# wagnva/semantic-nerf-for-satellite-data

Measured on AMD Instinct MI355X. Metric: train rays/sec (4096 rays x 64 samples), higher is better.
Workload: dtype f32(f16x2)

## Files before the change

### semantic-nerf-for-satellite-data_amd/csrc/bsp.h

```cpp
#pragma once
#include "common.h"
#include "gemm.h"

namespace snerf {
namespace bsp {

constexpr int RB = 128;
constexpr int CB = 128;
constexpr int E_MAX = 100;
constexpr int E_QUIET = 60;

typedef __amdgpu_buffer_rsrc_t srd_t;
typedef unsigned int u32x4 __attribute__((ext_vector_type(4)));
typedef unsigned int u32x2 __attribute__((ext_vector_type(2)));
typedef _Float16 f16x8 __attribute__((ext_vector_type(8)));
typedef _Float16 f16x4 __attribute__((ext_vector_type(4)));
constexpr unsigned OOB = 0xFFFFFFF0u;

__host__ __device__ inline int ncb_of(int ld) { return (ld + CB - 1) / CB; }
__host__ __device__ inline size_t plane_bytes(size_t rows, int ld, int pl = 2) { return rows * (size_t)ld * 2 * pl; }
__host__ __device__ inline size_t etab_ints(size_t rows, int ld) { return ((rows + RB - 1) / RB) * (size_t)ncb_of(ld); }
__host__ __device__ inline unsigned g16_off(int k, int pl = 2) { return (unsigned)(k >> 4) * 32u * (unsigned)pl + (unsigned)(k & 15) * 2u; }

__host__ __device__ inline int exp_of_maxbits(unsigned b) {
// ... 66 lines not shown
  const char* W = nullptr;
  const int* EW = nullptr;
  int w_rb32 = 0, w_row0 = 0, w_k0 = 0; unsigned w_bytes = 0;
  int I = 0, J = 0, K = 0;
  char* C = nullptr; int* EC = nullptr; int ldc = 0; int c_col0 = 0;
  float* Cf = nullptr;
  const float* bias = nullptr;
  int act = ACT_NONE; float w0 = 1.f;
  unsigned* Csign = nullptr;
  int aux_mode = AUX_NONE;
  const char* H = nullptr; const int* EH = nullptr; int ldh = 0; int h_col0 = 0; const unsigned* Hsign = nullptr;
  float* colsum = nullptr; int ldcs = 0;
  int tiles_i = 0, tiles_j = 0;
  int tj_skip = -1;
  int tiles_jr = 0;
  int rev = 0;
  int dbg = 0;
  int* tile_ctr = nullptr;
  int pl = 2;
  const float* nd_w = nullptr; float* nd_out = nullptr; unsigned long long nd_stride = 0;
  int nd_omax = 0, nd_ldw = 0;
  int nd_rows[8] = {0, 0, 0, 0, 0, 0, 0, 0}, nd_row0[8] = {0, 0, 0, 0, 0, 0, 0, 0}, nd_woff[8] = {0, 0, 0, 0, 0, 0, 0, 0};
};
__host__ __device__ inline size_t sign_words(size_t rows, int ld) { return ((rows + 31) / 32) * (size_t)((ld + 63) / 64) * 64; }

struct DwArgs {
  const char* A = nullptr; const int* EA = nullptr; int lda = 0; int a_col0 = 0;
  const char* B = nullptr; const int* EB = nullptr; int ldb = 0; int b_col0 = 0;
  int I = 0, J = 0, P = 0;
  float* C = nullptr; int ldc = 0;
  int k_split = 0, n_split = 1; unsigned long long slab_stride = 0;
  int tiles_i = 0, tiles_j = 0;
  int pl = 2;
};

constexpr int TR_MAXL = 8;
constexpr int TR_SLOTS = TR_MAXL + 1;
struct TrunkArgs {
  const char* pe = nullptr; const int* Epe = nullptr;
  int P = 0, W = 0, L = 0; unsigned skip_mask = 0;
  int gamma_free_layer = 0;
  const char* Wp[TR_SLOTS] = {}; const int* EW[TR_SLOTS] = {}; unsigned w_bytes[TR_SLOTS] = {}; int K[TR_SLOTS] = {};
  const float* bias[TR_SLOTS] = {}; float w0[TR_SLOTS] = {};
  char* F = nullptr; int* EF = nullptr; int ldf = 0;
  char* H[TR_MAXL] = {}; int* EH[TR_MAXL] = {}; unsigned* Hsign[TR_MAXL] = {};
  const float* nd_w = nullptr; float* nd_out = nullptr; unsigned long long nd_stride = 0;
  int* tile_ctr = nullptr;
  int dbg = 0;
};
inline int trunk_gamma_free_layer(int L, unsigned skip_mask) {
  int g = 2;
  for (int l = 2; l < L; ++l)
    if ((skip_mask >> l) & 1u) g = l;
  return g < L - 1 ? g : L - 1;
}
inline bool trunk_dma_in_final_layer(int L, unsigned skip_mask, bool feats_fused) {
  return !feats_fused && trunk_gamma_free_layer(L, skip_mask) == L - 1;
}
int launch_trunk(const TrunkArgs& a, bool train, hipStream_t st);
void trunk_set_grid_override(int n);
void trunk_set_fusion(int on);
bool trunk_fusion_enabled();

int launch_kc(const KcArgs& a, hipStream_t st);
void kc_set_grid_override(int n);
int launch_kc_narrow(const KcArgs& a, hipStream_t st);
// ... 48 lines not shown
```

### semantic-nerf-for-satellite-data_amd/csrc/bsp_gemm.hip

```cpp
#include "bsp_dev.h"

#include <vector>

namespace snerf {
namespace bsp {

constexpr int KC_STRIP = 32 * 68 * 4;
constexpr int KN_A = 128 * 64, KN_RING = 4, KN_TAIL = KN_RING * KN_A, KN_LDS = KN_TAIL + 512;

template <int PL>
__global__ __launch_bounds__(256, 4) void gemm_kcn_kernel(const KcArgs p) {
  constexpr int EB = 2 * PL, KSUB = PL == 2 ? 16 : 32, KSH = PL == 2 ? 4 : 5;
  __shared__ __attribute__((aligned(16))) char lds[KN_LDS];
  int* etab = reinterpret_cast<int*>(lds + KN_TAIL);
  const int t = threadIdx.x, lane = t & 63;
  const int wave = __builtin_amdgcn_readfirstlane(t >> 6);
  const int ti = blockIdx.x, i0 = ti * 128, wi0 = wave * 32;
  const int nks16 = p.K >> 4;
  const int nks = (p.K + KSUB - 1) >> KSH, nks1 = nks;
  const srd_t srdA = make_srd(p.A + ((size_t)i0 * p.lda + p.a_col0) * EB,
                              clamp_bytes(i0 < p.I ? ((unsigned long long)(p.I - i0 - 1) * p.lda + p.Ka) * (unsigned long long)EB : 0ull));
  const srd_t srdW = make_srd(p.W, p.w_bytes);
  unsigned voA[2];
#pragma unroll
// ... 39 lines not shown
  const unsigned fo0 = (unsigned)rowl * 64u + (unsigned)(((0 + kh) ^ swz) << 4);
  const unsigned fo1 = (unsigned)rowl * 64u + (unsigned)(((2 + kh) ^ swz) << 4);
  auto step = [&](int s, int slot, BFrag& bc, BFrag& bn) {
    wait_vm<2>();
    barrier_raw();
    if (__builtin_expect(((s < 64 ? chg0 >> s : chg1 >> (s - 64)) & 1ull) != 0ull, 0)) acc = scale_acc(acc, etab[s] - etab[s - 1]);
    loadB(s + 1, bn);
    issueA(s + 2, (slot + 2) % KN_RING);
    const char* st = lds + slot * KN_A;
    if constexpr (PL == 2) {
      acc = mfma3(ldsfrag(st + wi0 * 64 + fo0), ldsfrag(st + wi0 * 64 + fo1), __builtin_bit_cast(f16x8, bc.h), __builtin_bit_cast(f16x8, bc.l), acc);
    } else {
      acc = __builtin_amdgcn_mfma_f32_32x32x16_f16(ldsfrag(st + wi0 * 64 + fo0), __builtin_bit_cast(f16x8, bc.h), acc, 0, 0, 0);
      acc = __builtin_amdgcn_mfma_f32_32x32x16_f16(ldsfrag(st + wi0 * 64 + fo1), __builtin_bit_cast(f16x8, bc.l), acc, 0, 0, 0);
    }
  };
  for (int s = 0; s < nks; s += 4) {
    step(s, 0, bq0, bq1);
    if (s + 1 < nks) step(s + 1, 1, bq1, bq0);
    if (s + 2 < nks) step(s + 2, 2, bq0, bq1);
    if (s + 3 < nks) step(s + 3, 3, bq1, bq0);
  }
  wait_vm<0>();
  const int e_in = e_last + *p.EW;
  const int col = wf16_row(lane & 31);
  const float bj = (p.bias != nullptr && col < p.J) ? p.bias[col] : 0.f;
#pragma unroll
  for (int r = 0; r < 16; ++r) {
    const int row = i0 + wi0 + (r & 3) + 8 * (r >> 2) + 4 * (lane >> 5);
    if (row < p.I && col < p.J) p.Cf[(size_t)row * 32 + col] = __builtin_amdgcn_ldexpf(acc[r], -e_in) + bj;
  }
}

template <int TI, int PL> struct DwCfg {
  static constexpr int NTH = TI == 256 ? 512 : 256, WAVES = NTH / 64;
  static constexpr int MI = TI == 256 ? 4 : 1;
  static constexpr int EB = 2 * PL;
  static constexpr int PTS = PL == 2 ? 16 : 32;
  static constexpr int SPC = 128 / PTS;
  static constexpr int A_PITCH = TI * EB;
  static constexpr int B_PITCH = 256 * EB;
  static constexpr int A_BYTES = PTS * A_PITCH, B_BYTES = PTS * B_PITCH, STAGE = A_BYTES + B_BYTES, RING = 3;
  static constexpr int STRIPS = WAVES * KC_STRIP;
  static constexpr int TAIL = (RING * STAGE > STRIPS) ? RING * STAGE : STRIPS;
  static constexpr int MAXCH = 128;
  static constexpr int DUMMY = TAIL + WAVES * MAXCH * 4;
  static constexpr int LDS = DUMMY + (TI == 256 ? 0 : WAVES * 1024);
};
template <int PITCH> __device__ __forceinline__ unsigned dw_swz(int p) {
  return PITCH == 1024 ? (unsigned)(((p & 1) << 5) | ((p & 2) << 6)) : (PITCH == 512 ? (unsigned)((p & 3) << 6) : (PITCH == 128 ? (unsigned)((p & 2) << 4) : 0u));
}

template <int TI, int PL>
__global__ __launch_bounds__(TI == 256 ? 512 : 256, 2) void gemm_dw_kernel(const DwArgs p) {
  using T = DwCfg<TI, PL>;
  constexpr int EB = T::EB, PTS = T::PTS;
  __shared__ __attribute__((aligned(16))) char lds[T::LDS];
  int* esum = reinterpret_cast<int*>(lds + T::TAIL);

  const int t = threadIdx.x, lane = t & 63;
  const int wave = __builtin_amdgcn_readfirstlane(t >> 6);
  const int wi0 = TI == 256 ? (wave >> 2) * 128 : 0, wj0 = (wave & 3) * 64;
  int tile, split;
  split_tile_of_block(blockIdx.x, blockIdx.z, gridDim.x, gridDim.z, tile, split);
  const int ti = tile / p.tiles_j, tj = tile - ti * p.tiles_j;
  const int i0 = ti * TI, j0 = tj * 256;
  const int kBeg = split * p.k_split, kEnd = min(p.P, kBeg + p.k_split);
  const int nks = (kEnd - kBeg + PTS - 1) / PTS;
  float* C = p.C + (size_t)split * p.slab_stride;

  const srd_words srdA = make_srd_words(p.A + ((size_t)kBeg * p.lda + p.a_col0 + i0) * EB,
                                        clamp_bytes(kEnd > kBeg ? ((unsigned long long)(kEnd - kBeg) * p.lda - (p.a_col0 + i0)) * (unsigned long long)EB : 0ull));
  const srd_words srdB = make_srd_words(p.B + ((size_t)kBeg * p.ldb + p.b_col0 + j0) * EB,
                                        clamp_bytes(kEnd > kBeg ? ((unsigned long long)(kEnd - kBeg) * p.ldb - (p.b_col0 + j0)) * (unsigned long long)EB : 0ull));
  const unsigned lds0 = __builtin_amdgcn_readfirstlane(lds_addr(lds));
  constexpr int PA = T::A_PITCH, PB = T::B_PITCH;
  constexpr int A_PIECES = T::A_BYTES / 1024;
  constexpr int NPA = (A_PIECES + T::WAVES - 1) / T::WAVES;
  constexpr int NPB = 16 / T::WAVES;
  constexpr int RPA = PA >= 1024 ? 1 : 1024 / PA, RPB = 1024 / PB;
  constexpr int LRA = 64 / RPA, LRB = 64 / RPB;
  unsigned voA[NPA], voB[NPB];
  int prA[NPA], prB[NPB];
#pragma unroll
  for (int q = 0; q < NPA; ++q) {
    const int piece = wave * NPA + q;
    const int pr = piece * RPA + lane / LRA;
    const unsigned byte = 16u * (unsigned)(lane % LRA);
    prA[q] = piece < A_PIECES ? pr : -1;
    voA[q] = (unsigned)pr * (unsigned)p.lda * (unsigned)EB + (byte ^ dw_swz<PA>(pr));
  }
#pragma unroll
  for (int q = 0; q < NPB; ++q) {
    const int piece = wave * NPB + q;
    const int pr = piece * RPB + lane / LRB;
    prB[q] = pr;
    voB[q] = (unsigned)pr * (unsigned)p.ldb * (unsigned)EB + ((16u * (unsigned)(lane % LRB)) ^ dw_swz<PB>(pr));
  }
  auto issue = [&](int s, int slot) {
    const int prow0 = kBeg + PTS * s;
#pragma unroll
    for (int q = 0; q < NPA; ++q) {
      const int piece = wave * NPA + q;
      const bool ok = s < nks && prA[q] >= 0 && prow0 + prA[q] < kEnd;
      dma16_asm(srdA, lds0 + (unsigned)(piece < A_PIECES ? slot * T::STAGE + piece * 1024 : T::DUMMY + wave * 1024), ok ? voA[q] : OOB,
                (unsigned)s * (unsigned)PTS * (unsigned)p.lda * (unsigned)EB);
    }
#pragma unroll
    for (int q = 0; q < NPB; ++q) {
      const bool ok = s < nks && prow0 + prB[q] < kEnd;
      dma16_asm(srdB, lds0 + (unsigned)(slot * T::STAGE + T::A_BYTES + (wave * NPB + q) * 1024), ok ? voB[q] : OOB, (unsigned)s * (unsigned)PTS * (unsigned)p.ldb * (unsigned)EB);
    }
  };
  const int nch = (kEnd - kBeg + 127) >> 7;
  {
    const int ncbA = ncb_of(p.lda), ncbB = ncb_of(p.ldb);
    const int cbA = min((p.a_col0 + i0 + wi0) >> 7, ncbA - 1), cbB = min((p.b_col0 + j0 + wj0) >> 7, ncbB - 1);
    for (int c = lane; c < nch; c += 64) {
      const size_t rb = (size_t)(kBeg >> 7) + c;
      esum[wave * T::MAXCH + c] = p.EA[rb * ncbA + cbA] + p.EB[rb * ncbB + cbB];
    }
  }

  issue(0, 0);
  issue(1, 1);
#pragma unroll
  for (int r = 2; r < T::RING - 1; ++r) issue(r, r);

  f32x16 acc[T::MI][2];
#pragma unroll
  for (int mi = 0; mi < T::MI; ++mi)
#pragma unroll
    for (int nj = 0; nj < 2; ++nj)
#pragma unroll
      for (int r = 0; r < 16; ++r) acc[mi][nj][r] = 0.f;

  const int g = lane >> 4, q4 = (lane >> 2) & 3, pp = lane & 3;
  const int kq = 8 * (g >> 1) + q4;
  auto frag_off = [&](int col, int pl, int pitch, unsigned sw) -> unsigned {
    if constexpr (PL == 2) return (unsigned)kq * (unsigned)pitch + ((((unsigned)(col >> 4) * 64u) + (unsigned)pl * 32u + 8u * (unsigned)pp) ^ sw);
    else return (unsigned)(kq + 16 * pl) * (unsigned)pitch + ((((unsigned)(col >> 4) * 32u) + 8u * (unsigned)pp) ^ sw);
  };
  unsigned foA[T::MI][2], foB[2][2];
#pragma unroll
  for (int mi = 0; mi < T::MI; ++mi)
#pragma unroll
    for (int pl = 0; pl < 2; ++pl) foA[mi][pl] = frag_off(wi0 + 32 * mi + 16 * (g & 1), pl, PA, dw_swz<PA>(q4));
#pragma unroll
  for (int nj = 0; nj < 2; ++nj)
#pragma unroll
    for (int pl = 0; pl < 2; ++pl) foB[nj][pl] = (unsigned)T::A_BYTES + frag_off(wj0 + 32 * nj + 16 * (g & 1), pl, PB, dw_swz<PB>(q4));
  typedef __fp16 h4_t __attribute__((__vector_size__(4 * sizeof(__fp16))));
  typedef h4_t __attribute__((address_space(3))) * lds4_t;
  auto trfrag = [&](const char* base, unsigned off, int pitch) -> f16x8 {
    const f16x4 a = __builtin_bit_cast(f16x4, __builtin_amdgcn_ds_read_tr16_b64_v4f16((lds4_t)(base + off)));
    const f16x4 b = __builtin_bit_cast(f16x4, __builtin_amdgcn_ds_read_tr16_b64_v4f16((lds4_t)(base + off + 4 * pitch)));
    return f16x8{a[0], a[1], a[2], a[3], b[0], b[1], b[2], b[3]};
  };

  int e_cur = 0;
  bool quiet = false;
  constexpr int NPIECE = NPA + NPB;
  auto mma = [](f16x8 ah, f16x8 al, f16x8 bh, f16x8 bl, f32x16 c) -> f32x16 {
    if constexpr (PL == 2) return mfma3(ah, al, bh, bl, c);
    c = __builtin_amdgcn_mfma_f32_32x32x16_f16(ah, bh, c, 0, 0, 0);
    return __builtin_amdgcn_mfma_f32_32x32x16_f16(al, bl, c, 0, 0, 0);
  };
  auto chunk = [&](int s) {
    if ((s & (T::SPC - 1)) != 0) return;
    const int e_new = __builtin_amdgcn_readfirstlane(esum[wave * T::MAXCH + s / T::SPC]);
    quiet = s != 0 && e_new - e_cur > 64;
    if (s == 0) e_cur = e_new;
    else if (__builtin_expect(e_new != e_cur && !quiet, 0)) {
      const int de = e_new - e_cur;
#pragma unroll
      for (int mi = 0; mi < T::MI; ++mi)
#pragma unroll
        for (int nj = 0; nj < 2; ++nj) acc[mi][nj] = scale_acc(acc[mi][nj], de);
      e_cur = e_new;
    }
  };
  const bool active = (j0 + wj0 < p.J) && (i0 + wi0 < p.I);
  if constexpr (TI == 256) {
    const int grp = wave >> 2;
    f16x8 fa_h[4], fa_l[4], fb_h[2], fb_l[2];
    auto phaseM = [&](int s, int slot) {
      issue(s + T::RING - 1, (slot + T::RING - 1) % T::RING);
      if (!active) return;
      chunk(s);
      const char* st = lds + slot * T::STAGE;
#pragma unroll
      for (int nj = 0; nj < 2; ++nj) { fb_h[nj] = trfrag(st, foB[nj][0], PB); fb_l[nj] = trfrag(st, foB[nj][1], PB); }
#pragma unroll
      for (int mi = 0; mi < 4; ++mi) { fa_h[mi] = trfrag(st, foA[mi][0], PA); fa_l[mi] = trfrag(st, foA[mi][1], PA); }
      if (__builtin_expect(quiet, 0)) {
#pragma unroll
        for (int nj = 0; nj < 2; ++nj) { fb_h[nj] = f16x8{}; fb_l[nj] = f16x8{}; }
      }
    };
    auto phaseC = [&]() {
      if (!active) return;
      __builtin_amdgcn_s_setprio(1);
#pragma unroll
      for (int mi = 0; mi < 4; ++mi)
#pragma unroll
        for (int nj = 0; nj < 2; ++nj) acc[mi][nj] = mma(fa_h[mi], fa_l[mi], fb_h[nj], fb_l[nj], acc[mi][nj]);
      __builtin_amdgcn_s_setprio(0);
    };
    wait_vm<(T::RING - 2) * NPIECE>();
    barrier_raw();
    if (grp == 0) {
      int slot = 0;
      for (int s = 0; s < nks; ++s) {
        phaseM(s, slot);
        barrier_raw();
        phaseC();
        wait_vm<(T::RING - 2) * NPIECE>();
        barrier_raw();
        slot = slot == T::RING - 1 ? 0 : slot + 1;
      }
      barrier_raw();
    } else {
      barrier_raw();
      int slot = 0;
      for (int s = 0; s < nks; ++s) {
        phaseM(s, slot);
        wait_vm<(T::RING - 2) * NPIECE>();
        barrier_raw();
        phaseC();
        barrier_raw();
        slot = slot == T::RING - 1 ? 0 : slot + 1;
      }
    }
  } else
  {
  auto step = [&](int s, int slot) {
    wait_vm<NPIECE>();
    barrier_raw();
    issue(s + T::RING - 1, (slot + T::RING - 1) % T::RING);
// ... 13 lines not shown
      for (int nj = 0; nj < 2; ++nj) acc[mi][nj] = mma(ah, al, bh[nj], bl[nj], acc[mi][nj]);
    }
  };
  for (int s = 0; s < nks; s += 3) {
    step(s, 0);
    if (s + 1 < nks) step(s + 1, 1);
    if (s + 2 < nks) step(s + 2, 2);
  }
  }
  wait_vm<0>();
  barrier_raw();

  float* strip = reinterpret_cast<float*>(lds + wave * KC_STRIP);
  const int lc = lane & 31, lh = lane >> 5;
  const int rrow = lane >> 4, c4 = (lane & 15) * 4;
  const int col = j0 + wj0 + c4;
  const size_t offC = uniform_sz((size_t)(i0 + wi0) * p.ldc + j0 + wj0);
  const srd_t srdC = make_srd(C + offC, 0xFFFFFFE0u);
#pragma unroll
  for (int mi = 0; mi < T::MI; ++mi) {
#pragma unroll
    for (int n = 0; n < 2; ++n)
#pragma unroll
      for (int r = 0; r < 16; ++r)
        strip[((r & 3) + 8 * (r >> 2) + 4 * lh) * 68 + 32 * n + lc] = __builtin_amdgcn_ldexpf(acc[mi][n][r], -e_cur);
#pragma unroll
    for (int ps = 0; ps < 8; ++ps) {
      const int rl = 32 * mi + rrow + 4 * ps;
      const bool ok = col < p.J && (i0 + wi0 + rl) < p.I;
      const float4 v = *reinterpret_cast<const float4*>(&strip[(rrow + 4 * ps) * 68 + c4]);
      const u32x4 d = {__float_as_uint(v.x), __float_as_uint(v.y), __float_as_uint(v.z), __float_as_uint(v.w)};
      __builtin_amdgcn_raw_buffer_store_b128(d, srdC, ok ? ((unsigned)rl * (unsigned)p.ldc + (unsigned)c4) * 4u : OOB, 0, 2);
      store_data_guard(d);
    }
  }
}

int prof_hook_begin(double flops, int variant, hipStream_t st);
void prof_hook_end(int token, hipStream_t st);

static int bad(const char* why) {
  set_error("bsp gemm: %s", why);
  return SNERF_ERR_BAD_DESC;
}

int check_kc(const KcArgs& a, bool narrow) {
  if (!a.A || !a.EA || !a.W || !a.EW) return bad("null operand");
  if (a.pl != 1 && a.pl != 2) return bad("planes: 1 or 2");
  const int EB = 2 * a.pl, stage = a.pl == 2 ? 32 : 64;
  if (a.I <= 0 || a.J <= 0 || a.K <= 0) return bad("empty problem");
  if ((a.K & 15) || (a.Ka & 15) || a.Ka <= 0 || a.Ka > a.K || a.K > 2048) return bad("K and Ka must be multiples of 16, K <= 2048");
  if ((a.lda & 15) || (a.a_col0 & 15) || a.a_col0 + a.Ka > a.lda) return bad("A segment does not fit its tensor (16-column groups)");
  if (a.Ka < a.K && (a.Ka % stage)) return bad("two A segments: the first must be a whole number of LDS stages (32 columns; one plane: 64)");
  if (a.pl == 1 && ((a.a_col0 & 31) || (a.Ka < a.K && (a.a2_col0 & 31)))) return bad("one plane: A segments start on a multiple of 32 columns");
  if (a.Ka < a.K && (!a.A2 || !a.EA2 || (a.lda2 & 15) || (a.a2_col0 & 15) || a.a2_col0 + (a.K - a.Ka) > a.lda2)) return bad("second A segment");
  if ((a.w_row0 & 31) || (a.w_k0 & 15) || a.w_rb32 <= 0) return bad("weight operand must start on a 32-row / 16-k unit");
  if ((size_t)128 * (a.lda > a.lda2 ? a.lda : a.lda2) * EB >= 0x7FFFFFFFull) return bad("leading dimension too large");
  if (((uintptr_t)a.A & 15) || ((uintptr_t)a.W & 15) || (a.A2 && ((uintptr_t)a.A2 & 15))) return bad("operands must be 16-byte aligned");
  if (narrow) {
    if (!a.Cf || a.J > 32 || a.Ka != a.K) return bad("narrow variant: fp32 output, J <= 32, one A segment");
    return SNERF_OK;
  }
  if (!a.C || !a.EC || (a.ldc & 15) || (a.c_col0 & 127) || (a.J & 15) || a.c_col0 + a.J > a.ldc) return bad("BSP output: ldc % 16, c_col0 % 128, J % 16");
  if (((uintptr_t)a.C & 15) || (a.bias && ((uintptr_t)a.bias & 15))) return bad("output / bias alignment");
  if (a.aux_mode != AUX_NONE) {
    if (a.aux_mode != AUX_SINREC && a.aux_mode != AUX_RELU_MASK) return bad("unsupported aux mode");
// ... 8 lines not shown
  }
  if ((size_t)128 * a.ldc * EB >= 0x7FFFFFFFull) return bad("ldc too large");
  return SNERF_OK;
}

int launch_kc_narrow(const KcArgs& a0, hipStream_t st) {
  KcArgs a = a0;
  if (a.Ka == 0) a.Ka = a.K;
  a.A2 = a.A; a.EA2 = a.EA; a.lda2 = a.lda; a.a2_col0 = a.a_col0;
  int rc = check_kc(a, true);
  if (rc) return rc;
  const int tok = prof_hook_begin(2.0 * a.I * 32.0 * a.K, 3, st);
  if (a.pl == 2) hipLaunchKernelGGL(gemm_kcn_kernel<2>, dim3((a.I + 127) / 128), dim3(256), 0, st, a);
  else hipLaunchKernelGGL(gemm_kcn_kernel<1>, dim3((a.I + 127) / 128), dim3(256), 0, st, a);
  SNERF_LAUNCH_CHECK();
  prof_hook_end(tok, st);
  return SNERF_OK;
}

int launch_dw(const DwArgs& a0, bool narrow_i, hipStream_t st) {
  DwArgs a = a0;
  if (!a.A || !a.EA || !a.B || !a.EB || !a.C) return bad("dW: null operand");
  if (a.I <= 0 || a.J <= 0 || a.P <= 0) return bad("dW: empty problem");
  if ((a.lda & 15) || (a.ldb & 15) || (a.a_col0 & 15) || (a.b_col0 & 15) || (a.J & 3) || (a.ldc & 3)) return bad("dW: leading dimensions / column offsets");
  if (a.k_split <= 0 || (a.k_split & 127) || a.k_split > 16384 || a.n_split < 1) return bad("dW: k_split must be a multiple of 128, <= 16384");
  if (a.pl != 1 && a.pl != 2) return bad("dW: planes: 1 or 2");
  if ((size_t)a.k_split * (a.lda > a.ldb ? a.lda : a.ldb) * 2 * a.pl >= 0xFFFFFFF0ull) return bad("dW: k_split * ld exceeds the 32-bit span");
  if (narrow_i ? (a.I > 32 || ((a.a_col0 & 127) + 32 > 128)) : ((a.a_col0 & 127) != 0)) return bad("dW: the A columns of a wave must lie in one exponent block");
  if (a.b_col0 & 63) return bad("dW: b_col0 % 64");
  if (((uintptr_t)a.A & 15) || ((uintptr_t)a.B & 15) || ((uintptr_t)a.C & 15)) return bad("dW: alignment");
  const int TI = narrow_i ? 32 : 256;
  a.tiles_i = (a.I + TI - 1) / TI;
  a.tiles_j = (a.J + 255) / 256;
  const dim3 grid(a.tiles_i * a.tiles_j, 1, a.n_split);
  const int tok = prof_hook_begin(2.0 * a.I * (double)a.J * a.P, narrow_i ? 3 : 2, st);
  if (narrow_i) { if (a.pl == 2) hipLaunchKernelGGL((gemm_dw_kernel<32, 2>), grid, dim3(256), 0, st, a); else hipLaunchKernelGGL((gemm_dw_kernel<32, 1>), grid, dim3(256), 0, st, a); }
  else { if (a.pl == 2) hipLaunchKernelGGL((gemm_dw_kernel<256, 2>), grid, dim3(512), 0, st, a); else hipLaunchKernelGGL((gemm_dw_kernel<256, 1>), grid, dim3(512), 0, st, a); }
  SNERF_LAUNCH_CHECK();
  prof_hook_end(tok, st);
  return SNERF_OK;
}

}
}
```

### semantic-nerf-for-satellite-data_amd/csrc/bsp_pass.hip

```cpp
#include "aux_kernels.h"
#include "bsp.h"
#include "composite.h"
#include "normals.h"
#include "plan.h"

namespace snerf {

namespace {
struct Ws {
  char* base;
  char* c(size_t off) const { return base + off; }
  float* f(size_t off) const { return reinterpret_cast<float*>(base + off); }
  int* i(size_t off) const { return reinterpret_cast<int*>(base + off); }
  unsigned* u(size_t off) const { return reinterpret_cast<unsigned*>(base + off); }
  void a(bsp::KcArgs& g, const PlaneT& t, int k, int col0 = 0) const { g.A = c(t.o); g.EA = i(t.e); g.lda = t.ld; g.a_col0 = col0; g.Ka = k; }
  void a2(bsp::KcArgs& g, const PlaneT& t) const { g.A2 = c(t.o); g.EA2 = i(t.e); g.lda2 = t.ld; }
  void out(bsp::KcArgs& g, const PlaneT& t, int col0 = 0) const { g.C = c(t.o); g.EC = i(t.e); g.ldc = t.ld; g.c_col0 = col0; g.Csign = t.s ? u(t.s) : nullptr; }
  void h(bsp::KcArgs& g, const PlaneT& t, int col0 = 0) const { g.H = c(t.o); g.EH = i(t.e); g.ldh = t.ld; g.h_col0 = col0; g.Hsign = t.s ? u(t.s) : nullptr; }
  void dz(bsp::DwArgs& g, const PlaneT& t) const { g.A = c(t.o); g.EA = i(t.e); g.lda = t.ld; g.a_col0 = 0; }
  void x(bsp::DwArgs& g, const PlaneT& t, int col0) const { g.B = c(t.o); g.EB = i(t.e); g.ldb = t.ld; g.b_col0 = col0; }
};
struct WOp { const char* W; const int* EW; int rb32; unsigned bytes; int K; };
WOp wop(const Plan& p, const float* pk, int job) {
  const char* planes = reinterpret_cast<const char*>(pk + p.n_fp32);
  const bsp::WPackJob& w = p.wj.j[job];
  return {planes + w.dst_off, reinterpret_cast<const int*>(planes + p.wp_bytes) + w.e_idx, (w.rows + 31) / 32,
          (unsigned)bsp::wp16_bytes(w.rows, w.K, p.pl), w.K};
}
void weights(bsp::KcArgs& g, const Plan& p, const float* pk, int job, int row0 = 0, int k0 = 0) {
  const WOp w = wop(p, pk, job);
  g.W = w.W; g.EW = w.EW; g.w_rb32 = w.rb32; g.w_bytes = w.bytes;
  g.w_row0 = row0; g.w_k0 = k0;
  g.pl = p.pl;
}
void narrow_parts(CompArgs& c, const Plan& p, const float* pk, const Ws& ws) {
  c.part_stride = p.Pp;
  if (p.nd_sig) { c.sig_part = ws.f(p.o_sigpart); c.n_sig_part = 4 * (p.W / 256); c.sig_bias = pk + p.b_fs + p.W; }
// ... 202 lines not shown
size_t bsp_rq_floats(const Plan& p) {
  RQ rq{nullptr, ~(size_t)0};
  BwdRegions r;
  take_regions(p, rq, r);
  return rq.used;
}

int backward_bsp(const Plan& p, const float* pk, const SnerfInputs* in, const SnerfOutGrads* go, float* gp, float* d_t, float* d_t_s,
                 void* workspace, hipStream_t st) {
  const Ws ws{(char*)workspace};
  const int P = p.P, W = p.W, H = p.H;
  const bool embed = p.embed_grad;
  int kcq = 0;
  auto launch_kc = [&](bsp::KcArgs& g) { g.rev = kcq & 1; g.tile_ctr = kcq < KCQ_SLOTS ? ws.i(p.o_kcq) + 16 * kcq++ : nullptr; return bsp::launch_kc(g, st); };
  RQ rq{ws.f(p.o_rq), p.rq_floats};
  BwdRegions r;
  take_regions(p, rq, r, embed);
  if (rq.over) { set_error("reduction arena too small (plan / pass mismatch)"); return SNERF_ERR_WORKSPACE; }
  auto dact = [&](bsp::KcArgs& g, const PlaneT& h, int col0 = 0, float w0 = 1.f) {
    ws.h(g, h, col0);
    if (p.siren) { g.aux_mode = AUX_SINREC; g.w0 = w0; }
    else g.aux_mode = AUX_RELU_MASK;
  };
  auto colsum = [&](bsp::KcArgs& g, float* cs, int width) { g.colsum = cs; g.ldcs = cs_ld(width); };
  auto bias_from_colsum = [&](const float* cs, int width, float* gout) { return red_add_col(rq.col, cs, (P + 127) / 128, (size_t)cs_ld(width), width, gout); };
  auto dw_gemm = [&](const DwMat& m, const PlaneT& dz, int I, bool narrow_i, const PlaneT& X, int x_col0, int J, size_t slab_off = 0) {
    bsp::DwArgs g;
    ws.dz(g, dz); ws.x(g, X, x_col0);
    g.I = I; g.J = J; g.P = P;
    g.C = m.slab + slab_off; g.ldc = m.ldw;
    g.k_split = m.sp.k_split; g.n_split = m.sp.ns; g.slab_stride = m.stride; g.pl = p.pl;
    return bsp::launch_dw(g, narrow_i, st);
  };
  auto dw_reduce = [&](const DwMat& m, size_t count, float* gout) { return red_add_elem(rq.elem, m.slab, m.sp.ns, m.stride, count, gout); };
  auto narrow_grad = [&](const float* dnar, float* part, const PlaneT& t, float* gout) {
    RC(bsp::launch_colsum32_bsp(dnar, P, part, ws.c(t.o), ws.i(t.e), p.pl, st));
    return red_add_col(rq.col, part, (P + 255) / 256, NARROW, NARROW, gout);
  };
  float* dsig = ws.f(p.o_dsig); float* dfin = ws.f(p.o_dfin); float* dsun = ws.f(p.o_dsun);
  if (embed && p.sc) {
    if (d_t) RC(launch_zero_bytes(d_t, (size_t)p.N * p.tau * sizeof(float), st));
    if (d_t_s && p.x_ts >= 0) RC(launch_zero_bytes(d_t_s, (size_t)p.N * p.tau * sizeof(float), st));
    return SNERF_OK;
  }
  CompBwdArgs b;
  CompArgs& c = b.f;
  c.N = p.N; c.S = p.S; c.H = H; c.C = p.C; c.sc = p.sc; c.sem_sigmoid = p.sem_sigmoid; c.has_sbeta = p.blk_sbeta >= 0;
  c.z = ws.f(p.o_z); c.sigo = ws.f(p.o_sigo); c.fino = ws.f(p.o_fino); c.suno = ws.f(p.o_suno);
  narrow_parts(c, p, pk, ws);
  c.sun_d = in->sun_d; c.sun_stride = in->sun_stride; c.sky = pk + p.sky;
  b.T = ws.f(p.o_T); b.rgbraw = ws.f(p.o_rgbraw);
  b.g_rgb = go->rgb; b.g_depth = go->depth; b.g_weights = go->weights; b.g_transparency = go->transparency;
  b.g_albedo = go->albedo; b.g_sun = go->sun; b.g_sky = go->sky; b.g_beta = go->beta; b.g_sigmas = go->sigmas;
  b.g_beta_s = go->beta_semantic; b.g_logits = go->semantic_logits;
  b.d_sigo = dsig; b.d_fino = dfin; b.d_suno = dsun; b.sky_slab = (p.sc || embed) ? nullptr : ws.f(p.o_skyslab);
  b.zero = ws.u(p.o_kcq); b.zero_n = KCQ_SLOTS * 16;
  RC(launch_composite_bwd(b, st));
  if (!p.sc && !embed)
    RC(red_add_col(rq.col, ws.f(p.o_skyslab), p.comp_blocks * 4, (size_t)p.sky_floats, p.sky_floats, gp + p.sky));


  const PlaneT dz1 = p.dza.view(p.h1w);
  const int sun_col = p.sc ? 0 : p.sun_col;
  if (!p.sc) {
    if (embed) RC(bsp::launch_colsum32_bsp(dfin, P, r.nar_fin, ws.c(p.pdfin.o), ws.i(p.pdfin.e), p.pl, st));
    else {
// ... 38 lines not shown
    if (p.compose_feats) g.ldcs = r.ld_cs1;
    RC(launch_kc(g));
    if (!p.compose_feats) RC(bias_from_colsum(r.cs_sun, H, gp + p.b_h1 + (size_t)p.sun_col));
  }
  auto transient_grads = [&]() {
    const bool want_t = d_t != nullptr, want_ts = d_t_s != nullptr && p.x_ts >= 0;
    if (p.sc) {
      if (want_t) RC(launch_zero_bytes(d_t, (size_t)p.N * p.tau * sizeof(float), st));
      if (want_ts) RC(launch_zero_bytes(d_t_s, (size_t)p.N * p.tau * sizeof(float), st));
    } else if (want_t || want_ts) {
      int b_lo = p.blk_beta, b_hi = p.blk_beta;
      auto use = [&](int blk, bool on) { if (on && blk >= 0) { if (blk < b_lo) b_lo = blk; if (blk > b_hi) b_hi = blk; } };
      use(p.blk_rgb, p.rgb_t); use(p.blk_sem, p.sem_t || p.sem_ts); use(p.blk_sbeta, true);
      const int k_lo = b_lo * H, k_n = (b_hi + 1 - b_lo) * H;
      float* dext = ws.f(p.o_dfin);
      bsp::KcArgs x;
      ws.a(x, dz1, k_n, k_lo); weights(x, p, pk, p.wj_th1, p.Wf, k_lo);
      x.I = P; x.J = p.Xp; x.K = k_n; x.Cf = dext;
      RC(bsp::launch_kc_narrow(x, st));
      if (want_t) RC(launch_ray_sum32(dext, p.x_t, p.N, p.S, p.tau, d_t, st));
      if (want_ts) RC(launch_ray_sum32(dext, p.x_ts, p.N, p.S, p.tau, d_t_s, st));
    }
    return (int)SNERF_OK;
  };
  if (embed) return transient_grads();
  PlaneT dz_cur = p.dza.view(W);
  PlaneT dz_nxt = p.dzb.view(W);
  const bool sig_live = !p.sc || go->weights != nullptr || go->transparency != nullptr || go->sigmas != nullptr;
  const PlaneT& hl = p.h[p.L - 1];
  bool uncompose = false;
  if (p.compose_feats) {
    const int r0 = p.sc ? p.sun_col : 0;
    const int nt = (P + 127) / 128, X = p.FA - W;
    RC(dw_gemm(r.w_h1, dz1, p.h1w, false, p.fa, 0, p.FA));
    RC(red_add_elem2d(rq.elem, r.w_h1.slab + W, r.w_h1.sp.ns, r.w_h1.stride, p.h1w, X, p.FA, gp + p.w_h1 + (size_t)r0 * p.FA + W, p.FA));
    RC(red_add_elem2d(rq.elem, r.w_h1.slab, r.w_h1.sp.ns, r.w_h1.stride, p.h1w, W, p.FA, r.w_h1.slab, p.FA));
    RC(red_store_last(rq.elem));
    RC(red_add_col(rq.col, r.cs_fin, nt, (size_t)r.ld_cs1, p.h1w, r.cs_fin));
    RC(red_store_last(rq.col));
    uncompose = true;
    RC(transient_grads());
    if (sig_live) {
      RC(narrow_grad(dsig, r.nar_sig, p.pdsig, gp + p.b_fs + W));
      RC(dw_gemm(r.w_fs, p.pdsig, NARROW, true, hl, 0, W));
      RC(dw_reduce(r.w_fs, (size_t)NARROW * W, gp + p.w_fs + (size_t)W * W));
    }
    { const PlaneT sw = dz_cur; dz_cur = dz_nxt; dz_nxt = sw; }
    bsp::KcArgs g;
    ws.a(g, dz1, p.h1w);
    if (sig_live) ws.a2(g, p.pdsig);
    weights(g, p, pk, p.wj_th1, 0, r0); g.I = P; g.J = W; g.K = sig_live ? p.h1w + NARROW : p.h1w;
    ws.out(g, dz_cur);
    dact(g, hl, 0, (p.L == 1) ? 30.f : 1.f);
    colsum(g, r.cs_hl, W);
    RC(launch_kc(g));
    RC(bias_from_colsum(r.cs_hl, W, gp + p.b_tr[p.L - 1]));
  }
  const PlaneT dfa = p.dzb.view(p.FA);
  if (!p.compose_feats) {
    const int r0 = p.sc ? p.sun_col : 0;
    RC(dw_gemm(r.w_h1, dz1, p.h1w, false, p.fa, 0, p.FA));
    RC(dw_reduce(r.w_h1, (size_t)p.h1w * p.FA, gp + p.w_h1 + (size_t)r0 * p.FA));
    bsp::KcArgs g;
    ws.a(g, dz1, p.h1w); weights(g, p, pk, p.wj_th1, 0, r0);
    g.I = P; g.J = W; g.K = p.h1w; ws.out(g, dfa);
    colsum(g, r.cs_fa, p.FA);
    RC(launch_kc(g));
    RC(red_add_col(rq.col, r.cs_fa, (P + 127) / 128, (size_t)cs_ld(p.FA), W, gp + p.b_fs));
    RC(transient_grads());
  }
  if (!p.compose_feats) {
    if (sig_live) RC(narrow_grad(dsig, r.nar_sig, p.pdsig, gp + p.b_fs + W));
    RC(dw_gemm(r.w_fs, dfa, W, false, hl, 0, W));
    if (sig_live) RC(dw_gemm(r.w_fs, p.pdsig, NARROW, true, hl, 0, W, (size_t)W * W));
    RC(dw_reduce(r.w_fs, (size_t)(sig_live ? W + NARROW : W) * W, gp + p.w_fs));
    bsp::KcArgs g;
    ws.a(g, dfa, W);
    if (sig_live) ws.a2(g, p.pdsig);
    weights(g, p, pk, p.wj_tfs); g.I = P; g.J = W; g.K = sig_live ? W + NARROW : W;
    ws.out(g, dz_cur);
    dact(g, hl, 0, (p.L == 1) ? 30.f : 1.f);
    colsum(g, r.cs_hl, W);
    RC(launch_kc(g));
    RC(bias_from_colsum(r.cs_hl, W, gp + p.b_tr[p.L - 1]));
  }
  for (int i = p.L - 1; i >= 0; --i) {
    const BwdRegions::Layer& t = r.tr[i];
    if (i > 0 && ((p.skip_mask >> i) & 1u)) {
      RC(dw_gemm(t.w_gamma, dz_cur, W, false, p.pe, 0, p.Ep));
      RC(dw_gemm(t.w, dz_cur, W, false, p.h[i - 1], 0, W));
      RC(red_add_elem2d(rq.elem, t.w_gamma.slab, t.w_gamma.sp.ns, t.w_gamma.stride, W, p.Ep, p.Ep, gp + p.w_tr[i], p.k_tr[i]));
      RC(red_add_elem2d(rq.elem, t.w.slab, t.w.sp.ns, t.w.stride, W, W, W, gp + p.w_tr[i] + p.Ep, p.k_tr[i]));
    } else {
      if (i == 0) RC(dw_gemm(t.w, dz_cur, W, false, p.pe, 0, p.Ep));
      else RC(dw_gemm(t.w, dz_cur, W, false, p.h[i - 1], 0, W));
      RC(dw_reduce(t.w, (size_t)W * p.k_tr[i], gp + p.w_tr[i]));
    }
    if (i == 0) break;
    bsp::KcArgs g;
    ws.a(g, dz_cur, W); weights(g, p, pk, p.wj_tt[i]);
    g.I = P; g.J = W; g.K = W; ws.out(g, dz_nxt);
    dact(g, p.h[i - 1], 0, (i - 1 == 0) ? 30.f : 1.f);
    colsum(g, t.cs, W);
    RC(launch_kc(g));
    RC(bias_from_colsum(t.cs, W, gp + p.b_tr[i - 1]));
    const PlaneT sw = dz_cur; dz_cur = dz_nxt; dz_nxt = sw;
  }
  RC(launch_reductions(rq.elem, rq.col, st));
  if (!uncompose) return SNERF_OK;
  {
    const size_t r0 = p.sc ? (size_t)p.sun_col : 0;
    bsp::SgTable tb;
    bsp::uncompose_jobs(tb, r.w_h1.slab, r.cs_fin, pk + p.w_h1 + r0 * p.FA, pk + p.w_fs, pk + p.b_fs,
                        gp + p.w_h1 + r0 * p.FA, gp + p.b_h1 + r0, gp + p.w_fs, gp + p.b_fs, W, p.FA, p.h1w);
    return bsp::launch_sgemm(tb, 32, st);
  }
}

int density_grad_bsp(const Plan& p, const float* pk, const SnerfInputs* in, const float* coef, double* grad_ray, float* grad_sample,
                     void* workspace, void* scratch, hipStream_t st) {
  const Ws ws{(char*)workspace};
  const NormalsScratch ns = normals_scratch(p);
  double* G = reinterpret_cast<double*>((char*)scratch + ns.o_G);
  double* wd = reinterpret_cast<double*>((char*)scratch + ns.o_wd);
// ... 58 lines not shown
```

Baseline: 170,500.

## Fuse narrow second B segment into the wide dW GEMM kernel

```diff
diff --git a/include/snerf_test_dw2.h b/include/snerf_test_dw2.h
--- /dev/null
+++ b/include/snerf_test_dw2.h
@@ -0,0 +1,16 @@
+#ifndef SNERF_TEST_DW2_H
+#define SNERF_TEST_DW2_H
+
+#include "snerf_hip.h"
+
+#ifdef __cplusplus
+extern "C" {
+#endif
+
+int snerf_test_bsp_dw2(const float* A, int lda_src, const float* B, int ldb_src, const float* B2, int ldb2_src, int P, int I, int J, int J2,
+                       int a_col0, int b_col0, int b2_col0, int k_split, float* C, int ldc, float* C2, int ldc2, void* stream);
+
+#ifdef __cplusplus
+}
+#endif
+#endif
diff --git a/semantic-nerf-for-satellite-data_amd/csrc/bsp.h b/semantic-nerf-for-satellite-data_amd/csrc/bsp.h
--- a/semantic-nerf-for-satellite-data_amd/csrc/bsp.h
+++ b/semantic-nerf-for-satellite-data_amd/csrc/bsp.h
@@ -122,6 +122,8 @@
   int k_split = 0, n_split = 1; unsigned long long slab_stride = 0;
   int tiles_i = 0, tiles_j = 0;
   int pl = 2;
+  const char* B2 = nullptr; const int* EB2 = nullptr; int ldb2 = 0; int b2_col0 = 0; int J2 = 0;
+  float* C2 = nullptr; int ldc2 = 0; unsigned long long slab_stride2 = 0;
 };
 
 constexpr int TR_MAXL = 8;
diff --git a/semantic-nerf-for-satellite-data_amd/csrc/bsp_gemm.hip b/semantic-nerf-for-satellite-data_amd/csrc/bsp_gemm.hip
--- a/semantic-nerf-for-satellite-data_amd/csrc/bsp_gemm.hip
+++ b/semantic-nerf-for-satellite-data_amd/csrc/bsp_gemm.hip
@@ -95,7 +95,7 @@
   }
 }
 
-template <int TI, int PL> struct DwCfg {
+template <int TI, int PL, bool XB = false> struct DwCfg {
   static constexpr int NTH = TI == 256 ? 512 : 256, WAVES = NTH / 64;
   static constexpr int MI = TI == 256 ? 4 : 1;
   static constexpr int EB = 2 * PL;
@@ -103,23 +103,26 @@
   static constexpr int SPC = 128 / PTS;
   static constexpr int A_PITCH = TI * EB;
   static constexpr int B_PITCH = 256 * EB;
-  static constexpr int A_BYTES = PTS * A_PITCH, B_BYTES = PTS * B_PITCH, STAGE = A_BYTES + B_BYTES, RING = 3;
+  static constexpr int B2_PITCH = 32 * EB;
+  static constexpr int A_BYTES = PTS * A_PITCH, B_BYTES = PTS * B_PITCH, B2_BYTES = XB ? PTS * B2_PITCH : 0, STAGE = A_BYTES + B_BYTES + B2_BYTES, RING = 3;
   static constexpr int STRIPS = WAVES * KC_STRIP;
   static constexpr int TAIL = (RING * STAGE > STRIPS) ? RING * STAGE : STRIPS;
   static constexpr int MAXCH = 128;
-  static constexpr int DUMMY = TAIL + WAVES * MAXCH * 4;
-  static constexpr int LDS = DUMMY + (TI == 256 ? 0 : WAVES * 1024);
+  static constexpr int DUMMY = TAIL + (XB ? 2 : 1) * WAVES * MAXCH * 4;
+  static constexpr int LDS = DUMMY + ((TI == 256 && !XB) ? 0 : WAVES * 1024);
 };
 template <int PITCH> __device__ __forceinline__ unsigned dw_swz(int p) {
   return PITCH == 1024 ? (unsigned)(((p & 1) << 5) | ((p & 2) << 6)) : (PITCH == 512 ? (unsigned)((p & 3) << 6) : (PITCH == 128 ? (unsigned)((p & 2) << 4) : 0u));
 }
 
-template <int TI, int PL>
+template <int TI, int PL, bool XB = false>
 __global__ __launch_bounds__(TI == 256 ? 512 : 256, 2) void gemm_dw_kernel(const DwArgs p) {
-  using T = DwCfg<TI, PL>;
+  static_assert(!XB || (TI == 256 && PL == 2), "the second B segment: 256-row tiles, two planes");
+  using T = DwCfg<TI, PL, XB>;
   constexpr int EB = T::EB, PTS = T::PTS;
   __shared__ __attribute__((aligned(16))) char lds[T::LDS];
   int* esum = reinterpret_cast<int*>(lds + T::TAIL);
+  int* esum2 = esum + T::WAVES * T::MAXCH;
 
   const int t = threadIdx.x, lane = t & 63;
   const int wave = __builtin_amdgcn_readfirstlane(t >> 6);
@@ -160,6 +163,19 @@
     prB[q] = pr;
     voB[q] = (unsigned)pr * (unsigned)p.ldb * (unsigned)EB + ((16u * (unsigned)(lane % LRB)) ^ dw_swz<PB>(pr));
   }
+  const int j20 = 32 * tj;
+  const int nj2 = XB ? min(max(p.J2 - j20, 0), 32) : 0;
+  srd_words srdB2 = {};
+  unsigned voB2 = OOB;
+  int prB2 = 0;
+  if constexpr (XB) {
+    srdB2 = make_srd_words(p.B2 + ((size_t)kBeg * p.ldb2 + p.b2_col0 + j20) * EB,
+                           clamp_bytes((kEnd > kBeg && nj2 > 0) ? ((unsigned long long)(kEnd - kBeg) * p.ldb2 - (p.b2_col0 + j20)) * (unsigned long long)EB : 0ull));
+    prB2 = (wave & 1) * 8 + (lane >> 3);
+    const unsigned sb = (16u * (unsigned)(lane & 7)) ^ dw_swz<T::B2_PITCH>(prB2);
+    const int cl = (int)(sb >> 6) * 16 + ((sb & 16u) ? 8 : 0);
+    if (wave < 2 && cl < nj2) voB2 = (unsigned)prB2 * (unsigned)p.ldb2 * (unsigned)EB + sb;
+  }
   auto issue = [&](int s, int slot) {
     const int prow0 = kBeg + PTS * s;
 #pragma unroll
@@ -173,6 +189,11 @@
     for (int q = 0; q < NPB; ++q) {
       const bool ok = s < nks && prow0 + prB[q] < kEnd;
       dma16_asm(srdB, lds0 + (unsigned)(slot * T::STAGE + T::A_BYTES + (wave * NPB + q) * 1024), ok ? voB[q] : OOB, (unsigned)s * (unsigned)PTS * (unsigned)p.ldb * (unsigned)EB);
+    }
+    if constexpr (XB) {
+      const bool ok = s < nks && prow0 + prB2 < kEnd;
+      dma16_asm(srdB2, lds0 + (unsigned)(wave < 2 ? slot * T::STAGE + T::A_BYTES + T::B_BYTES + wave * 1024 : T::DUMMY + wave * 1024), ok ? voB2 : OOB,
+                (unsigned)s * (unsigned)PTS * (unsigned)p.ldb2 * (unsigned)EB);
     }
   };
   const int nch = (kEnd - kBeg + 127) >> 7;
@@ -183,6 +204,13 @@
       const size_t rb = (size_t)(kBeg >> 7) + c;
       esum[wave * T::MAXCH + c] = p.EA[rb * ncbA + cbA] + p.EB[rb * ncbB + cbB];
     }
+    if constexpr (XB) {
+      const int ncbB2 = ncb_of(p.ldb2), cbB2 = min((p.b2_col0 + j20) >> 7, ncbB2 - 1);
+      for (int c = lane; c < nch; c += 64) {
+        const size_t rb = (size_t)(kBeg >> 7) + c;
+        esum2[wave * T::MAXCH + c] = p.EA[rb * ncbA + cbA] + p.EB2[rb * ncbB2 + cbB2];
+      }
+    }
   }
 
   issue(0, 0);
@@ -213,6 +241,16 @@
   for (int nj = 0; nj < 2; ++nj)
 #pragma unroll
     for (int pl = 0; pl < 2; ++pl) foB[nj][pl] = (unsigned)T::A_BYTES + frag_off(wj0 + 32 * nj + 16 * (g & 1), pl, PB, dw_swz<PB>(q4));
+  constexpr int PB2 = T::B2_PITCH;
+  const int cw = wave & 3;
+  unsigned foB2[2] = {0u, 0u};
+  f32x16 acc2;
+  if constexpr (XB) {
+#pragma unroll
+    for (int pl = 0; pl < 2; ++pl) foB2[pl] = (unsigned)(T::A_BYTES + T::B_BYTES) + frag_off(16 * (g & 1), pl, PB2, dw_swz<PB2>(q4));
+#pragma unroll
+    for (int r = 0; r < 16; ++r) acc2[r] = 0.f;
+  }
   typedef __fp16 h4_t __attribute__((__vector_size__(4 * sizeof(__fp16))));
   typedef h4_t __attribute__((address_space(3))) * lds4_t;
   auto trfrag = [&](const char* base, unsigned off, int pitch) -> f16x8 {
@@ -223,7 +261,7 @@
 
   int e_cur = 0;
   bool quiet = false;
-  constexpr int NPIECE = NPA + NPB;
+  constexpr int NPIECE = NPA + NPB + (XB ? 1 : 0);
   auto mma = [](f16x8 ah, f16x8 al, f16x8 bh, f16x8 bl, f32x16 c) -> f32x16 {
     if constexpr (PL == 2) return mfma3(ah, al, bh, bl, c);
     c = __builtin_amdgcn_mfma_f32_32x32x16_f16(ah, bh, c, 0, 0, 0);
@@ -243,31 +281,65 @@
       e_cur = e_new;
     }
   };
+  int e_cur2 = 0;
+  bool quiet2 = false;
+  auto chunk2 = [&](int s) {
+    if ((s & (T::SPC - 1)) != 0) return;
+    const int e_new = __builtin_amdgcn_readfirstlane(esum2[wave * T::MAXCH + s / T::SPC]);
+    quiet2 = s != 0 && e_new - e_cur2 > 64;
+    if (s == 0) e_cur2 = e_new;
+    else if (__builtin_expect(e_new != e_cur2 && !quiet2, 0)) {
+      acc2 = scale_acc(acc2, e_new - e_cur2);
+      e_cur2 = e_new;
+    }
+  };
   const bool active = (j0 + wj0 < p.J) && (i0 + wi0 < p.I);
+  const bool active2 = XB && nj2 > 0 && (i0 + wi0 + 32 * cw < p.I);
   if constexpr (TI == 256) {
     const int grp = wave >> 2;
-    f16x8 fa_h[4], fa_l[4], fb_h[2], fb_l[2];
+    f16x8 fa_h[4], fa_l[4], fb_h[2], fb_l[2], fb2_h, fb2_l;
     auto phaseM = [&](int s, int slot) {
       issue(s + T::RING - 1, (slot + T::RING - 1) % T::RING);
-      if (!active) return;
-      chunk(s);
+      if (!active && !active2) return;
       const char* st = lds + slot * T::STAGE;
-#pragma unroll
-      for (int nj = 0; nj < 2; ++nj) { fb_h[nj] = trfrag(st, foB[nj][0], PB); fb_l[nj] = trfrag(st, foB[nj][1], PB); }
+      if (active) {
+        chunk(s);
+#pragma unroll
+        for (int nj = 0; nj < 2; ++nj) { fb_h[nj] = trfrag(st, foB[nj][0], PB); fb_l[nj] = trfrag(st, foB[nj][1], PB); }
+      }
 #pragma unroll
       for (int mi = 0; mi < 4; ++mi) { fa_h[mi] = trfrag(st, foA[mi][0], PA); fa_l[mi] = trfrag(st, foA[mi][1], PA); }
-      if (__builtin_expect(quiet, 0)) {
+      if (active && __builtin_expect(quiet, 0)) {
 #pragma unroll
         for (int nj = 0; nj < 2; ++nj) { fb_h[nj] = f16x8{}; fb_l[nj] = f16x8{}; }
+      }
+      if constexpr (XB) {
+        if (active2) {
+          chunk2(s);
+          fb2_h = trfrag(st, foB2[0], PB2); fb2_l = trfrag(st, foB2[1], PB2);
+          if (__builtin_expect(quiet2, 0)) { fb2_h = f16x8{}; fb2_l = f16x8{}; }
+        }
       }
     };
     auto phaseC = [&]() {
-      if (!active) return;
+      if (!active && !active2) return;
       __builtin_amdgcn_s_setprio(1);
-#pragma unroll
-      for (int mi = 0; mi < 4; ++mi)
-#pragma unroll
-        for (int nj = 0; nj < 2; ++nj) acc[mi][nj] = mma(fa_h[mi], fa_l[mi], fb_h[nj], fb_l[nj], acc[mi][nj]);
+      if (active) {
+#pragma unroll
+        for (int mi = 0; mi < 4; ++mi)
+#pragma unroll
+          for (int nj = 0; nj < 2; ++nj) acc[mi][nj] = mma(fa_h[mi], fa_l[mi], fb_h[nj], fb_l[nj], acc[mi][nj]);
+      }
+      if constexpr (XB) {
+        if (active2) {
+          switch (cw) {
+            case 0: acc2 = mma(fa_h[0], fa_l[0], fb2_h, fb2_l, acc2); break;
+            case 1: acc2 = mma(fa_h[1], fa_l[1], fb2_h, fb2_l, acc2); break;
+            case 2: acc2 = mma(fa_h[2], fa_l[2], fb2_h, fb2_l, acc2); break;
+            default: acc2 = mma(fa_h[3], fa_l[3], fb2_h, fb2_l, acc2); break;
+          }
+        }
+      }
       __builtin_amdgcn_s_setprio(0);
     };
     wait_vm<(T::RING - 2) * NPIECE>();
@@ -347,6 +419,25 @@
       const u32x4 d = {__float_as_uint(v.x), __float_as_uint(v.y), __float_as_uint(v.z), __float_as_uint(v.w)};
       __builtin_amdgcn_raw_buffer_store_b128(d, srdC, ok ? ((unsigned)rl * (unsigned)p.ldc + (unsigned)c4) * 4u : OOB, 0, 2);
       store_data_guard(d);
+    }
+  }
+  if constexpr (XB) {
+    if (active2) {
+      const int rrow2 = lane >> 3, c42 = (lane & 7) * 4;
+      float* C2 = p.C2 + (size_t)split * p.slab_stride2;
+      const size_t offC2 = uniform_sz((size_t)(i0 + wi0 + 32 * cw) * p.ldc2 + j20);
+      const srd_t srdC2 = make_srd(C2 + offC2, 0xFFFFFFE0u);
+#pragma unroll
+      for (int r = 0; r < 16; ++r) strip[((r & 3) + 8 * (r >> 2) + 4 * lh) * 68 + lc] = __builtin_amdgcn_ldexpf(acc2[r], -e_cur2);
+#pragma unroll
+      for (int ps = 0; ps < 4; ++ps) {
+        const int rl = rrow2 + 8 * ps;
+        const bool ok = c42 < nj2 && (i0 + wi0 + 32 * cw + rl) < p.I;
+        const float4 v = *reinterpret_cast<const float4*>(&strip[rl * 68 + c42]);
+        const u32x4 d = {__float_as_uint(v.x), __float_as_uint(v.y), __float_as_uint(v.z), __float_as_uint(v.w)};
+        __builtin_amdgcn_raw_buffer_store_b128(d, srdC2, ok ? ((unsigned)rl * (unsigned)p.ldc2 + (unsigned)c42) * 4u : OOB, 0, 2);
+        store_data_guard(d);
+      }
     }
   }
 }
@@ -421,9 +512,23 @@
   const int TI = narrow_i ? 32 : 256;
   a.tiles_i = (a.I + TI - 1) / TI;
   a.tiles_j = (a.J + 255) / 256;
+  const bool xb = a.B2 != nullptr;
+  if (xb) {
+    if (narrow_i || a.pl != 2) return bad("dW: a second B segment needs 256-row tiles and two planes");
+    if (!a.EB2 || !a.C2) return bad("dW: second B segment: null operand");
+    if (a.J2 <= 0 || (a.J2 & 15) || a.J2 > 32 * a.tiles_j) return bad("dW: J2 must be a multiple of 16, at most 32 columns per column tile");
+    if ((a.ldb2 & 15) || (a.b2_col0 & 15) || a.b2_col0 + a.J2 > a.ldb2 || (a.ldc2 & 3) || a.J2 > a.ldc2 || (a.slab_stride2 & 3)) return bad("dW: second B segment: leading dimensions / column offset");
+    for (int tj = 0; 32 * tj < a.J2; ++tj) {
+      const int c0 = a.b2_col0 + 32 * tj, c1 = a.b2_col0 + (a.J2 < 32 * tj + 32 ? a.J2 : 32 * tj + 32) - 1;
+      if ((c0 >> 7) != (c1 >> 7)) return bad("dW: the 32 columns a tile takes of the second B segment must lie in one exponent block");
+    }
+    if ((size_t)a.k_split * a.ldb2 * 2 * a.pl >= 0xFFFFFFF0ull) return bad("dW: k_split * ldb2 exceeds the 32-bit span");
+    if (((uintptr_t)a.B2 & 15) || ((uintptr_t)a.C2 & 15)) return bad("dW: second B segment: alignment");
+  }
   const dim3 grid(a.tiles_i * a.tiles_j, 1, a.n_split);
-  const int tok = prof_hook_begin(2.0 * a.I * (double)a.J * a.P, narrow_i ? 3 : 2, st);
-  if (narrow_i) { if (a.pl == 2) hipLaunchKernelGGL((gemm_dw_kernel<32, 2>), grid, dim3(256), 0, st, a); else hipLaunchKernelGGL((gemm_dw_kernel<32, 1>), grid, dim3(256), 0, st, a); }
+  const int tok = prof_hook_begin(2.0 * a.I * (double)(a.J + (xb ? a.J2 : 0)) * a.P, narrow_i ? 3 : 2, st);
+  if (xb) hipLaunchKernelGGL((gemm_dw_kernel<256, 2, true>), grid, dim3(512), 0, st, a);
+  else if (narrow_i) { if (a.pl == 2) hipLaunchKernelGGL((gemm_dw_kernel<32, 2>), grid, dim3(256), 0, st, a); else hipLaunchKernelGGL((gemm_dw_kernel<32, 1>), grid, dim3(256), 0, st, a); }
   else { if (a.pl == 2) hipLaunchKernelGGL((gemm_dw_kernel<256, 2>), grid, dim3(512), 0, st, a); else hipLaunchKernelGGL((gemm_dw_kernel<256, 1>), grid, dim3(512), 0, st, a); }
   SNERF_LAUNCH_CHECK();
   prof_hook_end(tok, st);
diff --git a/semantic-nerf-for-satellite-data_amd/csrc/bsp_pass.hip b/semantic-nerf-for-satellite-data_amd/csrc/bsp_pass.hip
--- a/semantic-nerf-for-satellite-data_amd/csrc/bsp_pass.hip
+++ b/semantic-nerf-for-satellite-data_amd/csrc/bsp_pass.hip
@@ -3,6 +3,8 @@
 #include "composite.h"
 #include "normals.h"
 #include "plan.h"
+
+#include <cstdlib>
 
 namespace snerf {
 
@@ -271,6 +273,29 @@
     g.k_split = m.sp.k_split; g.n_split = m.sp.ns; g.slab_stride = m.stride; g.pl = p.pl;
     return bsp::launch_dw(g, narrow_i, st);
   };
+  const bool xb_on = [&] { const char* ev = getenv("SNERF_DW_XB"); return p.pl == 2 && !(ev && atoi(ev) == 0); }();
+  auto xb_fits = [&](int J, int x2_col0, int J2) {
+    if (!xb_on || J2 <= 0 || (J2 & 15) || (x2_col0 & 15) || J2 > 32 * ((J + 255) / 256)) return false;
+    for (int c = 0; c < J2; c += 32)
+      if (((x2_col0 + c) >> 7) != ((x2_col0 + (J2 < c + 32 ? J2 : c + 32) - 1) >> 7)) return false;
+    return true;
+  };
+  auto dw_gemm_xb = [&](const DwMat& m, const PlaneT& dz, int I, const PlaneT& X, int J, const PlaneT& X2, int x2_col0, int J2,
+                        float* c2, int ldc2, size_t stride2) {
+    bsp::DwArgs g;
+    ws.dz(g, dz); ws.x(g, X, 0);
+    g.I = I; g.J = J; g.P = P;
+    g.C = m.slab; g.ldc = m.ldw;
+    g.k_split = m.sp.k_split; g.n_split = m.sp.ns; g.slab_stride = m.stride; g.pl = p.pl;
+    g.B2 = ws.c(X2.o); g.EB2 = ws.i(X2.e); g.ldb2 = X2.ld; g.b2_col0 = x2_col0; g.J2 = J2;
+    g.C2 = c2; g.ldc2 = ldc2; g.slab_stride2 = stride2;
+    return bsp::launch_dw(g, false, st);
+  };
+  auto dw_head1 = [&](const PlaneT& dz1v) {
+    if (xb_fits(W, W, p.FA - W))
+      return dw_gemm_xb(r.w_h1, dz1v, p.h1w, p.fa, W, p.fa, W, p.FA - W, r.w_h1.slab + W, p.FA, r.w_h1.stride);
+    return dw_gemm(r.w_h1, dz1v, p.h1w, false, p.fa, 0, p.FA);
+  };
   auto dw_reduce = [&](const DwMat& m, size_t count, float* gout) { return red_add_elem(rq.elem, m.slab, m.sp.ns, m.stride, count, gout); };
   auto narrow_grad = [&](const float* dnar, float* part, const PlaneT& t, float* gout) {
     RC(bsp::launch_colsum32_bsp(dnar, P, part, ws.c(t.o), ws.i(t.e), p.pl, st));
@@ -375,7 +400,7 @@
   if (p.compose_feats) {
     const int r0 = p.sc ? p.sun_col : 0;
     const int nt = (P + 127) / 128, X = p.FA - W;
-    RC(dw_gemm(r.w_h1, dz1, p.h1w, false, p.fa, 0, p.FA));
+    RC(dw_head1(dz1));
     RC(red_add_elem2d(rq.elem, r.w_h1.slab + W, r.w_h1.sp.ns, r.w_h1.stride, p.h1w, X, p.FA, gp + p.w_h1 + (size_t)r0 * p.FA + W, p.FA));
     RC(red_add_elem2d(rq.elem, r.w_h1.slab, r.w_h1.sp.ns, r.w_h1.stride, p.h1w, W, p.FA, r.w_h1.slab, p.FA));
     RC(red_store_last(rq.elem));
@@ -402,7 +427,7 @@
   const PlaneT dfa = p.dzb.view(p.FA);
   if (!p.compose_feats) {
     const int r0 = p.sc ? p.sun_col : 0;
-    RC(dw_gemm(r.w_h1, dz1, p.h1w, false, p.fa, 0, p.FA));
+    RC(dw_head1(dz1));
     RC(dw_reduce(r.w_h1, (size_t)p.h1w * p.FA, gp + p.w_h1 + (size_t)r0 * p.FA));
     bsp::KcArgs g;
     ws.a(g, dz1, p.h1w); weights(g, p, pk, p.wj_th1, 0, r0);
@@ -430,9 +455,13 @@
   for (int i = p.L - 1; i >= 0; --i) {
     const BwdRegions::Layer& t = r.tr[i];
     if (i > 0 && ((p.skip_mask >> i) & 1u)) {
-      RC(dw_gemm(t.w_gamma, dz_cur, W, false, p.pe, 0, p.Ep));
-      RC(dw_gemm(t.w, dz_cur, W, false, p.h[i - 1], 0, W));
-      RC(red_add_elem2d(rq.elem, t.w_gamma.slab, t.w_gamma.sp.ns, t.w_gamma.stride, W, p.Ep, p.Ep, gp + p.w_tr[i], p.k_tr[i]));
+      const bool xb = xb_fits(W, 0, p.Ep) && t.w.sp.ns <= t.w_gamma.sp.ns;
+      if (xb) RC(dw_gemm_xb(t.w, dz_cur, W, p.h[i - 1], W, p.pe, 0, p.Ep, t.w_gamma.slab, p.Ep, t.w_gamma.stride));
+      else {
+        RC(dw_gemm(t.w_gamma, dz_cur, W, false, p.pe, 0, p.Ep));
+        RC(dw_gemm(t.w, dz_cur, W, false, p.h[i - 1], 0, W));
+      }
+      RC(red_add_elem2d(rq.elem, t.w_gamma.slab, xb ? t.w.sp.ns : t.w_gamma.sp.ns, t.w_gamma.stride, W, p.Ep, p.Ep, gp + p.w_tr[i], p.k_tr[i]));
       RC(red_add_elem2d(rq.elem, t.w.slab, t.w.sp.ns, t.w.stride, W, W, W, gp + p.w_tr[i] + p.Ep, p.k_tr[i]));
     } else {
       if (i == 0) RC(dw_gemm(t.w, dz_cur, W, false, p.pe, 0, p.Ep));
```

After: 170,500 (median of 3 runs). Within noise of the previous version (+0.0%).
